# ADharaUTEXAS123007/PhysicsBasedFWI2

Hardware: AMD Instinct MI355X
Metric: grid-cells*timesteps/sec (forward+adjoint gradient pass) (higher is better)
Workload: dtype f32; 1 GPU; elastic_marmousi2_100x300_32shots_3000steps; shots_per_gpu=32, nt=3000, parallelism=shots x1, kernel_family=forward: single launch, 8 slabs/shot; adjoint: single launch, 8 slabs/shot, snapshots=f32, cells=interior

## Files before the change

### include/mifwi.h

```cpp
#ifndef MIFWI_H
#define MIFWI_H

#include <stddef.h>
#include <stdint.h>

#ifdef __cplusplus
extern "C" {
#endif

#define MIFWI_VERSION_MAJOR 0
#define MIFWI_VERSION_MINOR 7

enum {
    MIFWI_OK = 0,
    MIFWI_EINVAL = -1,
    MIFWI_ENODEVICE = -2,
    MIFWI_EHIP = -3,
    MIFWI_ECFL = -4,
    MIFWI_ENOMEM = -5
};

const char *mifwi_last_error(void);
int mifwi_version(void);
int64_t mifwi_fallback_count(void);
// ... 68 lines not shown
enum { MIFWI_SNAPSHOT_F32 = 0, MIFWI_SNAPSHOT_BF16 = 1 };

typedef struct {
    int32_t gp, pitch, ngroups, shots_per_group;
    int64_t coef_elems;
    int64_t state_elems;
    int64_t work_forward_elems;
    int64_t work_backward_elems;
    int64_t snap_step_elems;
    int32_t snapshot_format;
    int32_t kernel_flags;
} mifwi_elastic_layout;

enum { MIFWI_EL_KERNEL_FWD_SINGLE_LAUNCH = 1, MIFWI_EL_KERNEL_ADJ_SINGLE_LAUNCH = 2, MIFWI_EL_KERNEL_FWD_FUSED_STEP = 4,
       MIFWI_EL_KERNEL_ADJ_FUSED_STEP = 8,
       MIFWI_EL_KERNEL_FWD_LANE_HALO = 16, MIFWI_EL_KERNEL_ADJ_LANE_HALO = 32 };

typedef struct mifwi_elastic_plan mifwi_elastic_plan;

int mifwi_elastic_plan_create(mifwi_elastic_plan **plan, int device,
                              const mifwi_elastic_desc *desc);
int mifwi_elastic_plan_destroy(mifwi_elastic_plan *plan);
int mifwi_elastic_plan_layout(const mifwi_elastic_plan *plan, mifwi_elastic_layout *out);
int mifwi_elastic_plan_pass_sizes(const mifwi_elastic_plan *plan, int32_t *forward_shots, int32_t *adjoint_groups);

int mifwi_elastic_plan_bind_pressure(mifwi_elastic_plan *plan, float *rec_p, const float *g_p);

int mifwi_elastic_forward(mifwi_elastic_plan *plan, const float *mat, const float *pz,
                          const float *px, const float *f, const int32_t *src_cell,
                          const float *src_w, const int32_t *rec_cell, const float *rec_w,
                          float *rec_vx, float *rec_vz, float *snap, float *work, int32_t n_begin,
                          int32_t n_end, int32_t flags, void *stream);

int mifwi_elastic_backward(mifwi_elastic_plan *plan, const float *mat, const float *pz,
                           const float *px, const int32_t *src_cell, const float *src_w,
                           const int32_t *rec_cell, const float *rec_w, const float *g_vx,
                           const float *g_vz, const float *snap, int32_t snap_first,
                           float *grad_mat, float *grad_f, float *work, int32_t n_hi, int32_t n_lo,
// ... 40 lines not shown
```

### physicsbasedfwi2_amd/_lib.py

```python
import ctypes
import os

_HERE = os.path.dirname(os.path.abspath(__file__))
LIB_PATH = os.environ.get("MIFWI_LIB") or os.path.join(_HERE, "libmifwi.so")

MIFWI_OK = 0
ZERO_STATE = 1
FINALIZE = 2
_ERR_NAMES = {-1: "EINVAL", -2: "ENODEVICE", -3: "EHIP", -4: "ECFL", -5: "ENOMEM"}


class MifwiError(RuntimeError):
    pass


class AcousticDesc(ctypes.Structure):
    _fields_ = [("n0", ctypes.c_int32), ("n1", ctypes.c_int32), ("nt", ctypes.c_int32),
                ("nshot", ctypes.c_int32), ("nsrc", ctypes.c_int32), ("nrec", ctypes.c_int32),
                ("ntap", ctypes.c_int32), ("c0", ctypes.c_float), ("c1", ctypes.c_float),
                ("shots_per_group", ctypes.c_int32), ("edge_rows", ctypes.c_int32),
                ("cpml_width", ctypes.c_int32)]


class AcousticLayout(ctypes.Structure):
# ... 10 lines not shown
                ("free_surface", ctypes.c_int32), ("shots_per_group", ctypes.c_int32),
                ("source_type", ctypes.c_int32), ("record_pressure", ctypes.c_int32),
                ("snapshot_format", ctypes.c_int32), ("fd_order", ctypes.c_int32)]


class ElasticLayout(ctypes.Structure):
    _fields_ = [("gp", ctypes.c_int32), ("pitch", ctypes.c_int32), ("ngroups", ctypes.c_int32),
                ("shots_per_group", ctypes.c_int32), ("coef_elems", ctypes.c_int64),
                ("state_elems", ctypes.c_int64), ("work_forward_elems", ctypes.c_int64),
                ("work_backward_elems", ctypes.c_int64), ("snap_step_elems", ctypes.c_int64),
                ("snapshot_format", ctypes.c_int32), ("kernel_flags", ctypes.c_int32)]


EL_KERNEL_FWD_SINGLE_LAUNCH, EL_KERNEL_ADJ_SINGLE_LAUNCH, EL_KERNEL_FWD_FUSED_STEP, EL_KERNEL_ADJ_FUSED_STEP = 1, 2, 4, 8
EL_KERNEL_FWD_LANE_HALO, EL_KERNEL_ADJ_LANE_HALO = 16, 32
SNAPSHOT_F32, SNAPSHOT_BF16 = 0, 1
_P = ctypes.c_void_p

SIGNATURES = {
    "mifwi_last_error": (ctypes.c_char_p, []),
    "mifwi_version": (ctypes.c_int, []),
    "mifwi_fallback_count": (ctypes.c_int64, []),
    "mifwi_agent_handoff_count": (ctypes.c_int64, []),
    "mifwi_slow_handoff_count": (ctypes.c_int64, []),
    "mifwi_device_count": (ctypes.c_int, []),
    "mifwi_device_info": (ctypes.c_int, [ctypes.c_int, _P, _P, _P]),
    "mifwi_acoustic_plan_create": (ctypes.c_int, [ctypes.POINTER(_P), ctypes.c_int,
                                                  ctypes.POINTER(AcousticDesc)]),
    "mifwi_acoustic_plan_destroy": (ctypes.c_int, [_P]),
    "mifwi_acoustic_plan_layout": (ctypes.c_int, [_P, ctypes.POINTER(AcousticLayout)]),
    "mifwi_acoustic_forward": (ctypes.c_int, [_P] * 12 + [ctypes.c_int32] * 3 + [_P]),
    "mifwi_acoustic_backward": (ctypes.c_int, [_P] * 10 + [ctypes.c_int32] + [_P] * 3 +
                                [ctypes.c_int32] * 3 + [_P]),
    "mifwi_elastic_plan_create": (ctypes.c_int, [ctypes.POINTER(_P), ctypes.c_int,
                                                 ctypes.POINTER(ElasticDesc)]),
    "mifwi_elastic_plan_destroy": (ctypes.c_int, [_P]),
    "mifwi_elastic_plan_layout": (ctypes.c_int, [_P, ctypes.POINTER(ElasticLayout)]),
    "mifwi_elastic_plan_bind_pressure": (ctypes.c_int, [_P, _P, _P]),
    "mifwi_elastic_plan_pass_sizes": (ctypes.c_int, [_P, _P, _P]),
    "mifwi_acoustic_plan_pass_sizes": (ctypes.c_int, [_P, _P, _P]),
    "mifwi_elastic_forward": (ctypes.c_int, [_P] * 13 + [ctypes.c_int32] * 3 + [_P]),
    "mifwi_elastic_backward": (ctypes.c_int, [_P] * 11 + [ctypes.c_int32] + [_P] * 3 +
                               [ctypes.c_int32] * 3 + [_P]),
    "mifwi_acoustic_born": (ctypes.c_int, [_P] * 8 + [ctypes.c_int32] + [_P] * 2 + [ctypes.c_int32] * 3 + [_P]),
    "mifwi_acoustic_plan_cluster_slabs": (ctypes.c_int, [_P, ctypes.c_int32]),
    "mifwi_elastic_plan_cluster_slabs": (ctypes.c_int, [_P, ctypes.c_int32]),
    "mifwi_misfit_work_elems": (ctypes.c_int64, [ctypes.c_int32, ctypes.c_int64, ctypes.c_int64]),
    "mifwi_misfit": (ctypes.c_int, [ctypes.c_int, ctypes.c_int32] + [_P] * 3 + [ctypes.c_int64] * 2 +
                     [_P] * 4),
    "mifwi_gradient_condition_work_elems": (ctypes.c_int64, [ctypes.c_int32]),
    "mifwi_gradient_condition": (ctypes.c_int, [ctypes.c_int] + [_P] * 3 + [ctypes.c_int32] * 3 + [_P, ctypes.c_float] +
                                 [ctypes.c_int32] * 2 + [_P] * 3),
    "mifwi_elastic_materials": (ctypes.c_int, [ctypes.c_int] + [_P] * 4 + [ctypes.c_int32] * 2 + [ctypes.c_float, ctypes.c_int32, _P]),
    "mifwi_elastic_materials_vjp": (ctypes.c_int, [ctypes.c_int] + [_P] * 7 + [ctypes.c_int32] * 2 +
# ... 50 lines not shown
```

### physicsbasedfwi2_amd/csrc/mifwi_elastic.hip

```cpp
#include "mifwi_common.h"

#include <vector>

#include <algorithm>
#include <cmath>
#include <cstdlib>

namespace {

constexpr int kThreads = 256;
#ifndef MIFWI_EL_MINWAVES
#define MIFWI_EL_MINWAVES 1
#endif
struct FdK { float c1, c2; };
inline FdK fd_weights(int order)
{
    return order == 2 ? FdK{1.0f, 0.0f} : FdK{(float)(9.0 / 8.0), (float)(-1.0 / 24.0)};
}

enum { F_VX = 0, F_VZ = 1, F_SXX = 2, F_SZZ = 3, F_SXZ = 4 };
enum { M_L = 0, M_M = 1, M_MU = 2, M_BX = 3, M_BZ = 4 };
enum { PA = 0, PB = 1, PK = 2, PAH = 3, PBH = 4, PKH = 5 };

struct ElParams {
// ... 1013 lines not shown
    int W, wl, xr0, wx, xcd;
    float *rec_p;
    const float *g_p;
    int snap_bf16;
    long long snap_shot;
    long long splane;
    int sblk;
    int pass_shots;
    int pass_groups;
    int fused;
    int fused_pass_shots;
    long long field_stride, shot_stride, fields_elems, psix_elems, psiz_elems, coef_elems;
    long long psi_elems;
    int cluster, NW, PL, fwd_PL, adj_PL, cl_shots, cl_lds, cl_ng;
    int cl_xh, adj_xh;
    int cl_adj, adj_NW, adj_shots, adj_lds, adj_ng, adj_zrows;
    long long xbuf_elems, list_elems, xcc_elems;
    long long tile_elems;
};

namespace {

ElParams el_base(const mifwi_elastic_plan *pl, const float *mat, const float *pz, const float *px)
{
    ElParams p;
    memset(&p, 0, sizeof(p));
    p.nz = pl->d.nz; p.nx = pl->d.nx; p.ng = pl->ng; p.gp = pl->gp; p.pitch = pl->pitch;
    p.field_stride = (unsigned)pl->field_stride; p.shot_stride = pl->shot_stride;
    p.nshot = pl->d.nshot; p.gs = 1;
    p.W = pl->W; p.wl = pl->wl; p.xr0 = pl->xr0; p.wx = pl->wx;
// ... 30 lines not shown
    int extra = 0;
    if (p.smp_out0 != nullptr && p.nsmp > 0)
        extra = mifwi::ceil_div(mifwi::ceil_div(p.gs * p.nsmp, kThreads), tiles_x);
    dim3 grid(tiles_x, p.tiles_z + extra, mifwi::ceil_div(nshot, p.gs)), block(kThreads);
    switch (pl->lx) {
        case 64: hipLaunchKernelGGL((el_step_s<64, 1, SAVE>), grid, block, 0, st, p); break;
        case 32: hipLaunchKernelGGL((el_step_s<32, 1, SAVE>), grid, block, 0, st, p); break;
        default: hipLaunchKernelGGL((el_step_s<16, 1, SAVE>), grid, block, 0, st, p); break;
    }
}

void el_cluster_setup(mifwi_elastic_plan *pl)
{
    pl->cluster = 0; pl->NW = 0; pl->PL = 4 * (pl->ng + 2); pl->cl_shots = 0;
    pl->cl_xh = 0; pl->adj_xh = 0;
    pl->adj_PL = pl->PL; pl->fwd_PL = pl->PL;
    const int skew = env_int("MIFWI_EL_PL_SKEW", 1);
    int Pskew = pl->ng + 2;
    while ((Pskew - pl->ng) % 16) ++Pskew;
    const int PL_plain = pl->PL;
    if (skew & 1) pl->PL = 4 * Pskew;
    if (skew & 2) pl->adj_PL = 4 * Pskew;
    pl->cl_lds = 0; pl->xbuf_elems = 0; pl->xcc_elems = 0;
    pl->cl_adj = 0; pl->adj_NW = 0; pl->adj_shots = 0; pl->adj_lds = 0; pl->adj_ng = 0; pl->adj_zrows = 0; pl->list_elems = 0;
    {
        const long long ntiles = (long long)mifwi::ceil_div(pl->ng, AGO) * mifwi::ceil_div(pl->d.nz, ATZ);
        pl->tile_elems = std::max<long long>(1024, mifwi::round_up64(pl->d.nshot * (2 * ntiles + 1 + (long long)pl->d.nrec * pl->d.ntap), 64));
    }
    if (pl->d.ntap != 1 || pl->d.source_type != 0 || pl->d.record_pressure) return;
    const bool want_fwd = env_int("MIFWI_EL_CLUSTER", 1) != 0;
// ... 11 lines not shown
            PLq = PL_plain;
            lds = (5LL * (rows + 4) * PLq + 6LL * pl->gp + 8LL * rows + 8) * sizeof(float);
        }
        if (lds > 150 * 1024) continue;
        if ((long long)rows * pl->ng > 2 * kEcThreads || kEcRowFields * pl->gp > kEcGr * kEcThreads) continue;
        const int per_launch = 8 * (ncu / (8 * nw));
        if (per_launch < 8) break;
        const double cost = mifwi::ceil_div(pl->d.nshot, per_launch) * (4.8 + (double)rows * pl->ng / kEcThreads);
        if (cost < best - 1e-9) {
            best = cost;
            pl->cluster = 1; pl->NW = nw; pl->cl_shots = per_launch; pl->cl_lds = (int)lds;
            pl->cl_ng = mifwi::ceil_div(rows * pl->ng, kEcThreads);
            pl->fwd_PL = PLq;
        }
    }
    auto xhalo_ok = [&](int nw, int ngq) {
        if (env_int("MIFWI_EL_XHALO", 1) == 0) return 0;
        for (int w = 0; w < nw; ++w) {
            int r0, R;
            ec_slab_rows(pl->d.nz, nw, w, r0, R);
            if (!ec_xhalo_deal_ok(R, pl->ng, ngq * kEcThreads)) return 0;
        }
        return 1;
    };
    pl->cl_xh = pl->cluster ? xhalo_ok(pl->NW, pl->cl_ng) : 0;
    if (pl->cluster) {
        for (const void *fn : {(const void *)el_cluster_fwd<false, 1, false>, (const void *)el_cluster_fwd<true, 1, false>,
                               (const void *)el_cluster_fwd<false, 2, false>, (const void *)el_cluster_fwd<true, 2, false>,
                               (const void *)el_cluster_fwd<false, 1, true>, (const void *)el_cluster_fwd<true, 1, true>,
                               (const void *)el_cluster_fwd<false, 2, true>, (const void *)el_cluster_fwd<true, 2, true>,
                               (const void *)el_cluster_fwd<false, 1, false, true>, (const void *)el_cluster_fwd<true, 1, false, true>,
                               (const void *)el_cluster_fwd<false, 2, false, true>, (const void *)el_cluster_fwd<true, 2, false, true>})
            if (hipFuncSetAttribute(fn, hipFuncAttributeMaxDynamicSharedMemorySize, mifwi::kClusterLdsLimit) != hipSuccess) {
                (void)hipGetLastError();
                pl->cluster = 0;
            }
    }
    const int forced_adj = env_int("MIFWI_EL_ADJ_NW", forced);
    if (env_int("MIFWI_EL_CLUSTER_ADJ", 1) != 0 && pl->d.shots_per_group <= 0) {
        double best_adj = 1e30;
// ... 19 lines not shown
            if (lds > kEaLdsLimit && PLq != PL_plain) {
                PLq = PL_plain;
                lds = adj_lds(PLq);
            }
            if (lds > kEaLdsLimit) continue;
            if ((long long)rows * pl->ng > 2 * kEcThreads || kEcRowFields * pl->gp > kEcGr * kEcThreads) continue;
            const int per_launch = 8 * (ncu / (8 * nw));
            if (per_launch < 8) break;
            const double cost = mifwi::ceil_div(pl->d.nshot, per_launch) * (4.8 + (double)rows * pl->ng / kEcThreads);
            if (cost < best_adj - 1e-9) {
                best_adj = cost;
                pl->cl_adj = 1; pl->adj_NW = nw; pl->adj_shots = per_launch; pl->adj_lds = (int)lds; pl->adj_PL = PLq;
                pl->adj_ng = mifwi::ceil_div(rows * pl->ng, kEcThreads); pl->adj_zrows = zmax;
            }
        }
        pl->adj_xh = pl->cl_adj ? xhalo_ok(pl->adj_NW, pl->adj_ng) : 0;
        if (pl->cl_adj)
            for (const void *fn : {(const void *)el_cluster_adj<1, false>, (const void *)el_cluster_adj<2, false>,
                                   (const void *)el_cluster_adj<1, true>, (const void *)el_cluster_adj<2, true>,
                                   (const void *)el_cluster_adj<1, false, true>, (const void *)el_cluster_adj<2, false, true>})
                if (hipFuncSetAttribute(fn, hipFuncAttributeMaxDynamicSharedMemorySize, kEaLdsLimit) != hipSuccess) {
                    (void)hipGetLastError();
                    pl->cl_adj = 0;
                }
    }
    const int nwmax = std::max(pl->cluster ? pl->NW : 0, pl->cl_adj ? pl->adj_NW : 0);
    pl->xcc_elems = nwmax > 0 ? mifwi::round_up64((long long)pl->d.nshot * nwmax, 64) : 0;
    if (nwmax > 0)
        pl->xbuf_elems = mifwi::round_up64(2LL * pl->d.nshot * nwmax * 4 * kEcRowFields * pl->gp, 64) + pl->xcc_elems + 64;
    if (pl->cl_adj)
        pl->list_elems = mifwi::round_up64((long long)pl->d.nshot * pl->adj_NW * (1 + pl->d.nrec), 64);
// ... 181 lines not shown
    }
    if (pl->cl_adj) {
        pl->gs = 1;
        pl->ngroups = d->nshot;
    }
    *plan = pl;
    return MIFWI_OK;
}

int mifwi_elastic_plan_cluster_slabs(const mifwi_elastic_plan *plan, int32_t adjoint)
{
    if (!plan) return 0;
    return adjoint ? (plan->cl_adj ? plan->adj_NW : 0) : (plan->cluster ? plan->NW : 0);
}

int mifwi_elastic_plan_pass_sizes(const mifwi_elastic_plan *plan, int32_t *forward_shots, int32_t *adjoint_groups)
{
    if (!plan) return mifwi::fail(MIFWI_EINVAL, "null plan");
    if (forward_shots) *forward_shots = plan->pass_shots;
    if (adjoint_groups) *adjoint_groups = plan->pass_groups;
    return MIFWI_OK;
}

int mifwi_elastic_plan_bind_pressure(mifwi_elastic_plan *plan, float *rec_p, const float *g_p)
{
    if (!plan) return mifwi::fail(MIFWI_EINVAL, "null plan");
    if ((rec_p || g_p) && !plan->d.record_pressure)
        return mifwi::fail(MIFWI_EINVAL, "the plan was created with record_pressure = 0");
    plan->rec_p = rec_p;
    plan->g_p = g_p;
// ... 5 lines not shown
    delete plan;
    return MIFWI_OK;
}

int mifwi_elastic_plan_layout(const mifwi_elastic_plan *pl, mifwi_elastic_layout *out)
{
    if (!pl || !out) return mifwi::fail(MIFWI_EINVAL, "null plan/layout");
    out->gp = pl->gp; out->pitch = pl->pitch; out->ngroups = pl->ngroups;
    out->shots_per_group = pl->gs;
    out->coef_elems = pl->coef_elems;
    out->snap_step_elems = pl->snap_shot * pl->d.nshot;
    out->snapshot_format = pl->snap_bf16 ? MIFWI_SNAPSHOT_BF16 : MIFWI_SNAPSHOT_F32;
    out->kernel_flags = (pl->cluster ? MIFWI_EL_KERNEL_FWD_SINGLE_LAUNCH : 0) | (pl->cl_adj ? MIFWI_EL_KERNEL_ADJ_SINGLE_LAUNCH : 0) |
                        (pl->fused ? MIFWI_EL_KERNEL_FWD_FUSED_STEP : 0) |
                        (pl->cluster && pl->cl_xh ? MIFWI_EL_KERNEL_FWD_LANE_HALO : 0) |
                        (pl->cl_adj && pl->adj_xh ? MIFWI_EL_KERNEL_ADJ_LANE_HALO : 0);
    const long long psi = pl->psi_elems;
    const long long bbox = mifwi::round_up64(4LL * pl->d.nshot, 64);
    out->state_elems = pl->fields_elems + psi;
    out->work_forward_elems = out->state_elems + bbox + (pl->cluster ? pl->xbuf_elems + out->state_elems : 0) +
                              (pl->fused ? out->state_elems : 0);
    const long long adj_state = pl->fields_elems + 2 * psi + 5LL * pl->ngroups * pl->splane;
    out->work_backward_elems = adj_state + bbox + (pl->cl_adj ? pl->xbuf_elems + pl->list_elems + adj_state : 0) +
                               pl->tile_elems;
    return MIFWI_OK;
}

int mifwi_elastic_forward(mifwi_elastic_plan *pl, const float *mat, const float *pz,
                          const float *px, const float *f, const int32_t *src_cell,
                          const float *src_w, const int32_t *rec_cell, const float *rec_w,
                          float *rec_vx, float *rec_vz, float *snap, float *work, int32_t n_begin,
// ... 28 lines not shown
        EcParams c;
        memset(&c, 0, sizeof(c));
        c.nz = d.nz; c.nx = d.nx; c.ng = pl->ng; c.gp = pl->gp; c.pitch = pl->pitch;
        c.field_stride = (unsigned)pl->field_stride; c.shot_stride = pl->shot_stride;
        c.nshot = d.nshot; c.NW = pl->NW; c.PL = pl->fwd_PL;
        c.n_first = n_begin; c.n_last = n_end;
        c.W = pl->W; c.wl = pl->wl; c.xr0 = pl->xr0; c.wx = pl->wx; c.fsurf = d.free_surface;
        c.psix_shot = 4LL * d.nz * pl->wx; c.psiz_shot = 4LL * 2 * pl->W * pl->gp;
        c.mat = mat; c.pz = pz; c.px = px;
        c.fields = fields; c.psix = psi_state; c.psiz = psi_state + pl->psix_elems;
        c.S = snap; c.s_first = n_begin; c.s_step = snap_step;
        c.nsrc = d.nsrc; c.nrec = d.nrec; c.src_cell = src_cell; c.src_w = src_w; c.f = f;
        c.rec_cell = rec_cell; c.rec_w = rec_w;
        c.rec_vx = want_rec ? rec_vx : nullptr; c.rec_vz = want_rec ? rec_vz : nullptr;
        c.dbg = env_int("MIFWI_EL_CL_DBG", 0);
        c.nap = env_int("MIFWI_POLL_NAP", mifwi::ceil_div(d.nz, c.NW) >= 8 ? 48 : 1);
        c.K = fd_weights(d.fd_order);
        float *backup = xbuf + pl->xbuf_elems;
        rc = el_cluster_backup(work, pl->fields_elems + psi, backup, flags, st);
        if (rc) return rc;
        rc = snap ? el_cluster_run<true, false>(pl, c, xbuf, st) : el_cluster_run<false, false>(pl, c, xbuf, st);
        if (rc == mifwi::kClusterMisplaced) {
            mifwi::note_agent_tier("elastic forward");
            rc = el_cluster_restore(work, pl->fields_elems + psi, backup, flags, st);
            if (rc) return rc;
            rc = snap ? el_cluster_run<true, true>(pl, c, xbuf, st) : el_cluster_run<false, true>(pl, c, xbuf, st);
        }
        if (rc != mifwi::kClusterTimedOut && rc != mifwi::kClusterMisplaced) return rc;
        mifwi::note_fallback("elastic");
        rc = el_cluster_restore(work, pl->fields_elems + psi, backup, flags, st);
// ... 154 lines not shown
        c.nshot = d.nshot; c.NW = pl->adj_NW; c.PL = pl->adj_PL;
        c.n_first = n_hi; c.n_last = n_lo; c.nt = d.nt;
        c.W = pl->W; c.wl = pl->wl; c.xr0 = pl->xr0; c.wx = pl->wx; c.fsurf = d.free_surface;
        c.zrows_max = pl->adj_zrows;
        c.psix_shot = 4LL * d.nz * pl->wx; c.psiz_shot = 4LL * 2 * pl->W * pl->gp; c.psix_elems = pl->psix_elems;
        c.mat = mat; c.pz = pz; c.px = px;
        c.fields = fields; c.psiA = psiA; c.psiB = psiB;
        c.S = snap; c.s_first = snap_first; c.s_step = snap_step;
        c.acc = acc;
        c.nsrc = d.nsrc; c.nrec = d.nrec; c.src_cell = src_cell; c.src_w = src_w;
        c.grad_f = want_f ? grad_f : nullptr;
        c.rec_cell = rec_cell; c.rec_w = rec_w; c.g_vx = g_vx; c.g_vz = g_vz;
        c.slab_cnt = lists; c.slab_list = lists + (long long)d.nshot * pl->adj_NW;
        c.rcv_direct = env_int("MIFWI_EL_ADJ_DIRECT", 1);
        c.dbg = env_int("MIFWI_EL_CL_DBG", 0);
        c.nap = env_int("MIFWI_POLL_NAP", mifwi::ceil_div(d.nz, c.NW) >= 8 ? 48 : 1);
        c.K = fd_weights(d.fd_order);
        c.xbuf = reinterpret_cast<unsigned long long *>(xbuf);
        c.err = reinterpret_cast<int *>(xbuf + pl->xbuf_elems - 64);
        c.xcc_tab = reinterpret_cast<int *>(xbuf + pl->xbuf_elems - 64 - pl->xcc_elems);
        const long long adj_state = pl->fields_elems + 2 * psi + nacc;
        float *backup = reinterpret_cast<float *>(lists) + pl->list_elems;
        rc = el_cluster_backup(work, adj_state, backup, flags, st);
        if (rc) return rc;
        auto attempt = [&](bool agent) -> int {
            MIFWI_HIP_TRY(hipMemsetAsync(xbuf, 0, sizeof(float) * pl->xbuf_elems, st));
#ifdef MIFWI_ABLATIONS
            const char *trace_path = getenv("MIFWI_EL_CL_TRACE");
            const size_t trace_n = 64 * 8 * 16;
            c.trace = nullptr;
// ... 107 lines not shown
```

### physicsbasedfwi2_amd/csrc/mifwi_elastic_cluster.h

```cpp
#pragma once

constexpr int kEcThreads = 512;
constexpr unsigned kEcMaxSpin = 400000;

struct EcParams {
    int nz, nx, ng, gp, pitch;
    unsigned field_stride;
    long long shot_stride;
    int nshot, NW, PL, shot0, shot1;
    int n_first, n_last;
    int W, wl, xr0, wx, fsurf;
    long long psix_shot, psiz_shot;
    const float *mat, *pz, *px;
    float *fields, *psix, *psiz;
    float *S;
    int s_first;
    long long s_step;
    int nsrc, nrec;
    const int *src_cell;
    const float *src_w, *f;
    const int *rec_cell;
    const float *rec_w;
    float *rec_vx, *rec_vz;
    unsigned long long *xbuf;
    int *err;
    int *xcc_tab;
    int dbg, nap;
    FdK K;
#ifdef MIFWI_ABLATIONS
    long long *trace;
#endif
};

#ifdef MIFWI_ABLATIONS
#define EC_STAMP(k)                                                                                        \
    do {                                                                                                   \
        if (p.trace && tr_on && it >= 64 && it < 128 && (t & 63) == 0)                                     \
            p.trace[((it - 64) * 8 + (t >> 6)) * 16 + (k)] = (long long)__builtin_readcyclecounter();      \
    } while (0)
#define EC_LAGGARD()                                                                                       \
    do {                                                                                                   \
        if ((kDbg(p) & 4096) && w == 1 && s == p.shot0 && (it & 63) == 1)                                  \
// ... 189 lines not shown
};

#ifndef EC_LATE_INTERIOR
#define EC_LATE_INTERIOR 1
#endif
#ifndef EA_PUBLISH_FIRST
#define EA_PUBLISH_FIRST 1
#endif
#ifndef EA_MATS_AHEAD_A
#define EA_MATS_AHEAD_A 0
#endif
#ifndef EA_MATS_AHEAD_C
#define EA_MATS_AHEAD_C 1
#endif
struct EcSlot { int lrw, g, cls; };
__host__ __device__ __forceinline__ EcSlot ec_slot(int v, int R, int ng, int slots)
{
    EcSlot s;
    s.lrw = 0; s.g = 0; s.cls = 0;
#if EC_LATE_INTERIOR
    const int nint = (R > 4 ? R - 4 : 0) * ng, nb = R * ng - nint;
    int b0 = (nint + 63) & ~63;
    if (b0 + nb > slots) b0 = nint;
    if (v < nint) {
        const int ir = v / ng;
        s.lrw = 2 + ir; s.g = v - ir * ng; s.cls = v < kEcThreads ? 1 : 3;
    } else if (v >= b0 && v < b0 + nb) {
        const int bi = v - b0, br = bi / ng;
        s.g = bi - br * ng;
        s.lrw = (R > 4 && br >= 2) ? R - 4 + br : br;
        s.cls = 2;
    }
#else
    if (v < R * ng) {
        s.lrw = v / ng; s.g = v - s.lrw * ng;
        s.cls = (s.lrw >= 2 && s.lrw < R - 2) ? 1 : 2;
    }
#endif
    return s;
}

constexpr int kNbL = 1, kNbR = 2, kNbFirst = 4, kNbLast = 8;
__host__ __device__ __forceinline__ int ec_nb(int v, int R, int ng, int slots)
{
    const EcSlot s = ec_slot(v, R, ng, slots);
    if (s.cls == 0) return 0;
    const int lane = v & 63;
    const bool lv = lane != 0 && ec_slot(v - 1, R, ng, slots).cls == s.cls;
    const bool rv = lane != 63 && ec_slot(v + 1, R, ng, slots).cls == s.cls;
    return (lv ? kNbL : 0) | (rv ? kNbR : 0) | (s.g == 0 ? kNbFirst : 0) | (s.g == ng - 1 ? kNbLast : 0);
}
inline bool ec_xhalo_deal_ok(int R, int ng, int slots)
{
    for (int v = 0; v < slots; ++v) {
        const EcSlot s = ec_slot(v, R, ng, slots);
        if (s.cls == 0) continue;
        const int nb = ec_nb(v, R, ng, slots), lane = v & 63;
        if (!(nb & (kNbL | kNbR))) return false;
        const int lc = lane != 0 ? ec_slot(v - 1, R, ng, slots).cls : 0;
        if (lc >= 2 && s.cls >= 2 && lc != s.cls) return false;
    }
    return true;
}
__device__ __forceinline__ float ec_lane_below(float old, float x)
{
    return __int_as_float(__builtin_amdgcn_update_dpp(__float_as_int(old), __float_as_int(x), 0x138, 0xf, 0xf, false));
}
__device__ __forceinline__ float ec_lane_above(float old, float x)
{
    return __int_as_float(__builtin_amdgcn_update_dpp(__float_as_int(old), __float_as_int(x), 0x130, 0xf, 0xf, false));
}
template <bool XH>
__device__ __forceinline__ void ec_xhalo(const float *q, const float4 &c, const int nb, const float *dummy, float2 &L, float2 &R)
{
    if (!XH) {
// ... 216 lines not shown
    int r0, R;
    ec_slab_rows(p.nz, p.NW, w, r0, R);
    const int PL = p.PL, LR = R + 4;
    const int fsz = LR * PL;
    EcCtx c;
    for (int k = 0; k < 5; ++k) c.Lf[k] = lds + ec_plane(k) * fsz;
    float *lpx = lds + 5 * fsz, *lpz = lpx + 6 * p.gp;
    c.lpx = lpx; c.lpz = lpz; c.PL = PL; c.fsurf = p.fsurf; c.K = p.K;
    const unsigned ncell = (unsigned)p.nz * p.gp;
    const float4 zero4 = make_float4(0.f, 0.f, 0.f, 0.f);
    const long long xplane = (long long)p.nz * p.wx, zplane = 2LL * p.W * p.gp;
    auto strip_x = [&](int g) { const int c0 = 4 * g; return p.W <= 0 ? -1 : c0 < p.wl ? c0 : c0 >= p.xr0 ? p.wl + (c0 - p.xr0) : -1; };
    auto strip_z = [&](int j) { return p.W <= 0 ? -1 : j < p.W ? j : j >= p.nz - p.W ? j - (p.nz - 2 * p.W) : -1; };

    EcGroup G[NG];
    bool slow = p.nrec > kEcThreads;
    int tsq = -1;
    unsigned tsrc4 = 0;
    unsigned tm0 = 0, tm1 = 0, tm2 = 0, tm3 = 0;
    float tw = 0.f, tnext = 0.f;
    int src_mask = 0;
#pragma unroll
    for (int q = 0; q < NG; ++q) {
        EcGroup &g = G[q];
        const EcSlot sl = ec_slot(t + q * kEcThreads, R, p.ng, NG * kEcThreads);
        const bool own = sl.cls != 0;
        const int lrw = sl.lrw;
        g.g = sl.g;
        g.j = r0 + lrw;
        g.cls = sl.cls;
        g.nb = XH ? ec_nb(t + q * kEcThreads, R, p.ng, NG * kEcThreads) : 0;
        g.lo = (lrw + 2) * PL + 4 + 4 * g.g;
        const unsigned gcc = (unsigned)g.j * p.gp + 4 * g.g;
        g.gcb = 4u * gcc;
        g.mL = g.mM = g.mMu = g.mBx = g.mBz = zero4;
        g.s1 = g.s2 = g.s3 = g.s4 = g.s5 = g.s6 = g.s7 = g.s8 = zero4;
        g.xtab = -1; g.ztab = -1;
        int xs_off = -1, zs = -1;
        if (own) {
            g.mL = ld4(p.mat + M_L * ncell + gcc); g.mM = ld4(p.mat + M_M * ncell + gcc);
            g.mMu = ld4(p.mat + M_MU * ncell + gcc);
            g.mBx = ld4(p.mat + M_BX * ncell + gcc); g.mBz = ld4(p.mat + M_BZ * ncell + gcc);
            xs_off = strip_x(g.g); zs = strip_z(g.j);
        }
        if (xs_off >= 0) {
            g.xtab = 24 * g.g;
            const float *q = p.psix + (long long)s * p.psix_shot + (long long)g.j * p.wx + xs_off;
            g.s1 = ld4(q); g.s3 = ld4(q + xplane); g.s5 = ld4(q + 2 * xplane); g.s8 = ld4(q + 3 * xplane);
        }
        if (zs >= 0) {
            g.ztab = 8 * lrw;
            const float *q = p.psiz + (long long)s * p.psiz_shot + (long long)zs * p.gp + 4 * g.g;
            g.s2 = ld4(q); g.s4 = ld4(q + zplane); g.s6 = ld4(q + 2 * zplane); g.s7 = ld4(q + 3 * zplane);
        }
        for (int e = 0; e < p.nsrc; ++e) {
            const int cell = p.src_cell[(long long)s * p.nsrc + e];
            if (cell < 0) continue;
            const int i0 = cell / p.nx, i1 = cell - i0 * p.nx;
            if (own && i0 == g.j && (i1 >> 2) == g.g) {
                if (tsq >= 0) slow = true;
                tw = p.src_w[(long long)s * p.nsrc + e];
                tsq = q; tsrc4 = 4u * e;
                tm0 = (i1 & 3) == 0 ? ~0u : 0u; tm1 = (i1 & 3) == 1 ? ~0u : 0u;
// ... 235 lines not shown
    int s_first;
    long long s_step;
    float *acc;
    int nsrc, nrec;
    const int *src_cell;
    const float *src_w;
    float *grad_f;
    const int *rec_cell;
    const float *rec_w, *g_vx, *g_vz;
    const int *slab_cnt, *slab_list;
    int rcv_direct;
    unsigned long long *xbuf;
    int *err;
    int *xcc_tab;
    int dbg, nap;
    FdK K;
#ifdef MIFWI_ABLATIONS
    long long *trace;
#endif
};

__global__ void ec_build_slab_lists(const int *rec_cell, int nrec, int nz, int nx, int NW, int *slab_cnt,
                                    int *slab_list)
{
    const int s = blockIdx.x;
    __shared__ int cnt[64];
    if ((int)threadIdx.x < NW) cnt[threadIdx.x] = 0;
    __syncthreads();
    const int base = nz / NW, rem = nz - base * NW;
    for (int e = threadIdx.x; e < nrec; e += blockDim.x) {
// ... 52 lines not shown
    const long long xplane = (long long)p.nz * p.wx, zplane = 2LL * p.W * p.gp;
    const int ztop_end = p.W > 0 ? min(r0 + R, p.W) : r0;
    const int ntop = max(0, ztop_end - r0);
    const int zbot_beg = p.W > 0 ? max(r0, p.nz - p.W) : r0 + R;
    const int zrows = ntop + max(0, r0 + R - zbot_beg);
    const int xsz = R * p.wx, zsz = zrows * p.gp;
    const int PL_ = PL, fsz_ = fsz, xsz_ = xsz, zsz_ = zsz;
    const unsigned ncell_ = ncell;

    const int par_in = (p.nt - 1 - p.n_first) & 1;
    const float *psi_in = par_in ? p.psiB : p.psiA;
    const int par_out = (p.nt - 1 - (p.n_last - 1)) & 1;
    float *psi_out = par_out ? p.psiB : p.psiA;

    EaGroup G[NG];
    bool slow = false;
#pragma unroll
    for (int q = 0; q < NG; ++q) {
        EaGroup &g = G[q];
        const EcSlot sl = ec_slot(t + q * kEcThreads, R, p.ng, NG * kEcThreads);
        const bool own = sl.cls != 0;
        const int lrw = sl.lrw;
        g.g = sl.g;
        g.j = r0 + lrw;
        g.lo = (lrw + 2) * PL + 4 + 4 * g.g;
        g.cls = sl.cls;
        g.nb = XH ? ec_nb(t + q * kEcThreads, R, p.ng, NG * kEcThreads) : 0;
        g.bxx = g.bzz = g.bxz = g.vx = g.vz = zero4;
        g.a0 = g.a1 = g.a2 = g.a3 = g.a4 = zero4;
        g.S1 = g.S2 = g.S3 = g.S4 = g.S5 = zero4;
        g.xsl = -1; g.zsl = -1; g.src = -1; g.src_wt = 0.f;
        if (own) {
            const unsigned gcc = (unsigned)g.j * p.gp + 4 * g.g;
            const long long o = (long long)(g.j + 2) * p.pitch + 4 + 4 * g.g;
            const float *gf = p.fields + (long long)s * p.shot_stride;
            g.vx = ld4(gf + F_VX * p.field_stride + o); g.vz = ld4(gf + F_VZ * p.field_stride + o);
            g.bxx = ld4(gf + F_SXX * p.field_stride + o); g.bzz = ld4(gf + F_SZZ * p.field_stride + o);
            g.bxz = ld4(gf + F_SXZ * p.field_stride + o);
            const float *ga = p.acc + (long long)s * 5 * ncell + gcc;
            g.a0 = ld4(ga); g.a1 = ld4(ga + ncell); g.a2 = ld4(ga + 2 * (long long)ncell);
            g.a3 = ld4(ga + 3 * (long long)ncell); g.a4 = ld4(ga + 4 * (long long)ncell);
            if (p.W > 0) {
                const int c0 = 4 * g.g;
                int xs_off = -1, zs = -1;
                if (c0 < p.wl) xs_off = c0; else if (c0 >= p.xr0) xs_off = p.wl + (c0 - p.xr0);
                if (g.j < p.W) zs = g.j; else if (g.j >= p.nz - p.W) zs = g.j - (p.nz - 2 * p.W);
                if (xs_off >= 0) {
                    g.xsl = lrw * p.wx + xs_off;
                    const float *qx = psi_in + (long long)s * p.psix_shot + (long long)g.j * p.wx + xs_off;
#pragma unroll
                    for (int k = 0; k < 4; ++k) st4(lxs + k * xsz + g.xsl, ld4(qx + k * xplane));
                }
                if (zs >= 0) {
                    const int zl = (g.j < p.W) ? g.j - r0 : ntop + (g.j - zbot_beg);
                    g.zsl = zl * p.gp + 4 * g.g;
                    const float *qz = psi_in + p.psix_elems + (long long)s * p.psiz_shot + (long long)zs * p.gp + 4 * g.g;
#pragma unroll
                    for (int k = 0; k < 4; ++k) st4(lzs + k * zsz + g.zsl, ld4(qz + k * zplane));
                }
            }
        }
        if (p.grad_f != nullptr)
            for (int e = 0; e < p.nsrc; ++e) {
                const int cell = p.src_cell[(long long)s * p.nsrc + e];
                if (cell < 0) continue;
                const int i0 = cell / p.nx, i1 = cell - i0 * p.nx;
// ... 510 lines not shown
```

Before: 68760 Mcells*steps/s.

## Deal PML strip groups into separate wavefront segments in cluster kernels

```diff
diff --git a/include/mifwi.h b/include/mifwi.h
--- a/include/mifwi.h
+++ b/include/mifwi.h
@@ -106,7 +106,8 @@
 
 enum { MIFWI_EL_KERNEL_FWD_SINGLE_LAUNCH = 1, MIFWI_EL_KERNEL_ADJ_SINGLE_LAUNCH = 2, MIFWI_EL_KERNEL_FWD_FUSED_STEP = 4,
        MIFWI_EL_KERNEL_ADJ_FUSED_STEP = 8,
-       MIFWI_EL_KERNEL_FWD_LANE_HALO = 16, MIFWI_EL_KERNEL_ADJ_LANE_HALO = 32 };
+       MIFWI_EL_KERNEL_FWD_LANE_HALO = 16, MIFWI_EL_KERNEL_ADJ_LANE_HALO = 32,
+       MIFWI_EL_KERNEL_FWD_STRIP_DEAL = 64, MIFWI_EL_KERNEL_ADJ_STRIP_DEAL = 128 };
 
 typedef struct mifwi_elastic_plan mifwi_elastic_plan;
 
@@ -114,6 +115,8 @@
                               const mifwi_elastic_desc *desc);
 int mifwi_elastic_plan_destroy(mifwi_elastic_plan *plan);
 int mifwi_elastic_plan_layout(const mifwi_elastic_plan *plan, mifwi_elastic_layout *out);
+int mifwi_elastic_deal_table(int32_t rows, int32_t groups, int32_t strip_left, int32_t strip_right, int32_t group_slots,
+                             int32_t mode, int32_t *table, int32_t *lane_halo_ok);
 int mifwi_elastic_plan_pass_sizes(const mifwi_elastic_plan *plan, int32_t *forward_shots, int32_t *adjoint_groups);
 
 int mifwi_elastic_plan_bind_pressure(mifwi_elastic_plan *plan, float *rec_p, const float *g_p);
diff --git a/physicsbasedfwi2_amd/_lib.py b/physicsbasedfwi2_amd/_lib.py
--- a/physicsbasedfwi2_amd/_lib.py
+++ b/physicsbasedfwi2_amd/_lib.py
@@ -48,6 +48,7 @@
 
 EL_KERNEL_FWD_SINGLE_LAUNCH, EL_KERNEL_ADJ_SINGLE_LAUNCH, EL_KERNEL_FWD_FUSED_STEP, EL_KERNEL_ADJ_FUSED_STEP = 1, 2, 4, 8
 EL_KERNEL_FWD_LANE_HALO, EL_KERNEL_ADJ_LANE_HALO = 16, 32
+EL_KERNEL_FWD_STRIP_DEAL, EL_KERNEL_ADJ_STRIP_DEAL = 64, 128
 SNAPSHOT_F32, SNAPSHOT_BF16 = 0, 1
 _P = ctypes.c_void_p
 
@@ -72,6 +73,7 @@
     "mifwi_elastic_plan_layout": (ctypes.c_int, [_P, ctypes.POINTER(ElasticLayout)]),
     "mifwi_elastic_plan_bind_pressure": (ctypes.c_int, [_P, _P, _P]),
     "mifwi_elastic_plan_pass_sizes": (ctypes.c_int, [_P, _P, _P]),
+    "mifwi_elastic_deal_table": (ctypes.c_int, [ctypes.c_int32] * 6 + [_P, _P]),
     "mifwi_acoustic_plan_pass_sizes": (ctypes.c_int, [_P, _P, _P]),
     "mifwi_elastic_forward": (ctypes.c_int, [_P] * 13 + [ctypes.c_int32] * 3 + [_P]),
     "mifwi_elastic_backward": (ctypes.c_int, [_P] * 11 + [ctypes.c_int32] + [_P] * 3 +
diff --git a/physicsbasedfwi2_amd/csrc/mifwi_elastic.hip b/physicsbasedfwi2_amd/csrc/mifwi_elastic.hip
--- a/physicsbasedfwi2_amd/csrc/mifwi_elastic.hip
+++ b/physicsbasedfwi2_amd/csrc/mifwi_elastic.hip
@@ -1051,6 +1051,8 @@
     long long psi_elems;
     int cluster, NW, PL, fwd_PL, adj_PL, cl_shots, cl_lds, cl_ng;
     int cl_xh, adj_xh;
+    int cl_deal, adj_deal;
+    int cl_seg, adj_seg;
     int cl_adj, adj_NW, adj_shots, adj_lds, adj_ng, adj_zrows;
     long long xbuf_elems, list_elems, xcc_elems;
     long long tile_elems;
@@ -1111,6 +1113,7 @@
 {
     pl->cluster = 0; pl->NW = 0; pl->PL = 4 * (pl->ng + 2); pl->cl_shots = 0;
     pl->cl_xh = 0; pl->adj_xh = 0;
+    pl->cl_deal = pl->adj_deal = pl->cl_seg = pl->adj_seg = 0;
     pl->adj_PL = pl->PL; pl->fwd_PL = pl->PL;
     const int skew = env_int("MIFWI_EL_PL_SKEW", 1);
     int Pskew = pl->ng + 2;
@@ -1152,16 +1155,27 @@
             pl->fwd_PL = PLq;
         }
     }
-    auto xhalo_ok = [&](int nw, int ngq) {
+    auto slab_deal = [&](int nw, int w, int ngq, int mode) {
+        int r0, R, gl, gr;
+        ec_slab_rows(pl->d.nz, nw, w, r0, R);
+        ec_strip_groups(pl->W, pl->wl, pl->xr0, pl->ng, mode, gl, gr);
+        return ec_deal(R, pl->ng, gl, gr, ngq * kEcThreads, mode);
+    };
+    auto xhalo_ok = [&](int nw, int ngq, int mode) {
         if (env_int("MIFWI_EL_XHALO", 1) == 0) return 0;
-        for (int w = 0; w < nw; ++w) {
-            int r0, R;
-            ec_slab_rows(pl->d.nz, nw, w, r0, R);
-            if (!ec_xhalo_deal_ok(R, pl->ng, ngq * kEcThreads)) return 0;
-        }
+        for (int w = 0; w < nw; ++w)
+            if (!ec_xhalo_deal_ok(slab_deal(nw, w, ngq, mode))) return 0;
         return 1;
     };
-    pl->cl_xh = pl->cluster ? xhalo_ok(pl->NW, pl->cl_ng) : 0;
+    auto pick_deal = [&](int nw, int ngq, int dflt, int &mode, int &xh, int &seg) {
+        mode = std::min(2, std::max(0, env_int("MIFWI_EL_DEAL", dflt)));
+        xh = xhalo_ok(nw, ngq, mode);
+        if (mode && !xh && xhalo_ok(nw, ngq, 0)) { mode = 0; xh = 1; }
+        seg = 0;
+        for (int w = 0; w < nw; ++w)
+            if (slab_deal(nw, w, ngq, mode).level > 0) seg = 1;
+    };
+    if (pl->cluster) pick_deal(pl->NW, pl->cl_ng, 0, pl->cl_deal, pl->cl_xh, pl->cl_seg);
     if (pl->cluster) {
         for (const void *fn : {(const void *)el_cluster_fwd<false, 1, false>, (const void *)el_cluster_fwd<true, 1, false>,
                                (const void *)el_cluster_fwd<false, 2, false>, (const void *)el_cluster_fwd<true, 2, false>,
@@ -1211,7 +1225,7 @@
                 pl->adj_ng = mifwi::ceil_div(rows * pl->ng, kEcThreads); pl->adj_zrows = zmax;
             }
         }
-        pl->adj_xh = pl->cl_adj ? xhalo_ok(pl->adj_NW, pl->adj_ng) : 0;
+        if (pl->cl_adj) pick_deal(pl->adj_NW, pl->adj_ng, 1, pl->adj_deal, pl->adj_xh, pl->adj_seg);
         if (pl->cl_adj)
             for (const void *fn : {(const void *)el_cluster_adj<1, false>, (const void *)el_cluster_adj<2, false>,
                                    (const void *)el_cluster_adj<1, true>, (const void *)el_cluster_adj<2, true>,
@@ -1423,6 +1437,22 @@
     return adjoint ? (plan->cl_adj ? plan->adj_NW : 0) : (plan->cluster ? plan->NW : 0);
 }
 
+int mifwi_elastic_deal_table(int32_t rows, int32_t groups, int32_t strip_left, int32_t strip_right, int32_t group_slots,
+                             int32_t mode, int32_t *table, int32_t *lane_halo_ok)
+{
+    if (rows < 1 || groups < 1 || strip_left < 0 || strip_right < 0 || group_slots < 1 || group_slots > 2 || !table ||
+        (long long)rows * groups > (long long)group_slots * kEcThreads)
+        return mifwi::fail(MIFWI_EINVAL, "bad deal shape %dx%d on %d group slots", rows, groups, group_slots);
+    const EcDeal d = ec_deal(rows, groups, strip_left, strip_right, group_slots * kEcThreads, mode);
+    for (int v = 0; v < d.slots; ++v) {
+        const EcSlot s = ec_slot(v, d);
+        table[4 * v] = s.cls ? s.lrw : -1; table[4 * v + 1] = s.cls ? s.g : -1;
+        table[4 * v + 2] = s.cls; table[4 * v + 3] = ec_nb(v, d);
+    }
+    if (lane_halo_ok) *lane_halo_ok = ec_xhalo_deal_ok(d) ? 1 : 0;
+    return d.level;
+}
+
 int mifwi_elastic_plan_pass_sizes(const mifwi_elastic_plan *plan, int32_t *forward_shots, int32_t *adjoint_groups)
 {
     if (!plan) return mifwi::fail(MIFWI_EINVAL, "null plan");
@@ -1458,7 +1488,9 @@
     out->kernel_flags = (pl->cluster ? MIFWI_EL_KERNEL_FWD_SINGLE_LAUNCH : 0) | (pl->cl_adj ? MIFWI_EL_KERNEL_ADJ_SINGLE_LAUNCH : 0) |
                         (pl->fused ? MIFWI_EL_KERNEL_FWD_FUSED_STEP : 0) |
                         (pl->cluster && pl->cl_xh ? MIFWI_EL_KERNEL_FWD_LANE_HALO : 0) |
-                        (pl->cl_adj && pl->adj_xh ? MIFWI_EL_KERNEL_ADJ_LANE_HALO : 0);
+                        (pl->cl_adj && pl->adj_xh ? MIFWI_EL_KERNEL_ADJ_LANE_HALO : 0) |
+                        (pl->cluster && pl->cl_seg ? MIFWI_EL_KERNEL_FWD_STRIP_DEAL : 0) |
+                        (pl->cl_adj && pl->adj_seg ? MIFWI_EL_KERNEL_ADJ_STRIP_DEAL : 0);
     const long long psi = pl->psi_elems;
     const long long bbox = mifwi::round_up64(4LL * pl->d.nshot, 64);
     out->state_elems = pl->fields_elems + psi;
@@ -1517,6 +1549,7 @@
         c.rec_cell = rec_cell; c.rec_w = rec_w;
         c.rec_vx = want_rec ? rec_vx : nullptr; c.rec_vz = want_rec ? rec_vz : nullptr;
         c.dbg = env_int("MIFWI_EL_CL_DBG", 0);
+        c.deal = pl->cl_deal;
         c.nap = env_int("MIFWI_POLL_NAP", mifwi::ceil_div(d.nz, c.NW) >= 8 ? 48 : 1);
         c.K = fd_weights(d.fd_order);
         float *backup = xbuf + pl->xbuf_elems;
@@ -1701,6 +1734,7 @@
         c.slab_cnt = lists; c.slab_list = lists + (long long)d.nshot * pl->adj_NW;
         c.rcv_direct = env_int("MIFWI_EL_ADJ_DIRECT", 1);
         c.dbg = env_int("MIFWI_EL_CL_DBG", 0);
+        c.deal = pl->adj_deal;
         c.nap = env_int("MIFWI_POLL_NAP", mifwi::ceil_div(d.nz, c.NW) >= 8 ? 48 : 1);
         c.K = fd_weights(d.fd_order);
         c.xbuf = reinterpret_cast<unsigned long long *>(xbuf);
diff --git a/physicsbasedfwi2_amd/csrc/mifwi_elastic_cluster.h b/physicsbasedfwi2_amd/csrc/mifwi_elastic_cluster.h
--- a/physicsbasedfwi2_amd/csrc/mifwi_elastic_cluster.h
+++ b/physicsbasedfwi2_amd/csrc/mifwi_elastic_cluster.h
@@ -26,6 +26,7 @@
     int *err;
     int *xcc_tab;
     int dbg, nap;
+    int deal;
     FdK K;
 #ifdef MIFWI_ABLATIONS
     long long *trace;
@@ -245,11 +246,61 @@
 #define EA_MATS_AHEAD_C 1
 #endif
 struct EcSlot { int lrw, g, cls; };
-__host__ __device__ __forceinline__ EcSlot ec_slot(int v, int R, int ng, int slots)
-{
+struct EcDeal {
+    int R, ng, gl, gr, slots;
+    int level;
+    int is0, b0, bs0;
+};
+__host__ __device__ __forceinline__ EcDeal ec_deal(int R, int ng, int gl, int gr, int slots, int mode)
+{
+    EcDeal d;
+    d.R = R; d.ng = ng; d.gl = gl; d.gr = gr; d.slots = slots;
+    d.level = 0; d.is0 = d.b0 = d.bs0 = 0;
+    const int nn = ng - gl - gr, ns = gl + gr, ri = R - 4;
+    if (mode <= 0 || ns <= 0 || nn < 2 || ri < 1) return d;
+    d.is0 = (ri * (nn + 1) - 1 + 63) & ~63;
+    d.b0 = (d.is0 + ri * (ns + 1) + 63) & ~63;
+    const int bn = 4 * (nn + 1) - 1, bs = 4 * (ns + 1);
+    const int nint = ri * ng, nbnd = 4 * ng;
+    const int plain = ((nint + 63) & ~63) + nbnd <= slots ? ((nint + 63) >> 6) + ((nbnd + 63) >> 6) : (nint + nbnd + 63) >> 6;
+    const int ws3 = (((d.b0 + bn + 63) & ~63) + bs + 63) >> 6, ws2 = (d.b0 + bn + 1 + bs + 63) >> 6, ws1 = (d.b0 + nbnd + 63) >> 6;
+    if (mode >= 2 && ws3 <= plain && ws3 * 64 <= slots) { d.level = 3; d.bs0 = (d.b0 + bn + 63) & ~63; }
+    else if (mode >= 2 && ws2 <= plain && ws2 * 64 <= slots) { d.level = 2; d.bs0 = d.b0 + bn + 1; }
+    else if (ws1 <= plain && ws1 * 64 <= slots) d.level = 1;
+    return d;
+}
+__host__ __device__ __forceinline__ EcSlot ec_slot(int v, const EcDeal &d)
+{
+    const int R = d.R, ng = d.ng, slots = d.slots;
     EcSlot s;
     s.lrw = 0; s.g = 0; s.cls = 0;
+    if (v < 0 || v >= slots) return s;
 #if EC_LATE_INTERIOR
+    if (d.level > 0) {
+        const int nn = ng - d.gl - d.gr, ns = d.gl + d.gr, ri = R - 4;
+        int row = -1, g = 0;
+        if (v < d.is0) {
+            const int r = v / (nn + 1), k = v - r * (nn + 1);
+            if (r < ri && k < nn) { row = r; g = d.gl + k; }
+        } else if (v < d.b0) {
+            const int u = v - d.is0, r = u / (ns + 1), k = u - r * (ns + 1);
+            if (r < ri && k != d.gl) { row = r; g = k < d.gl ? k : ng - d.gr + (k - d.gl - 1); }
+        } else if (d.level == 1) {
+            const int u = v - d.b0, r = u / ng;
+            if (r < 4) { row = ri + r; g = u - r * ng; }
+        } else if (v < d.bs0) {
+            const int u = v - d.b0, r = u / (nn + 1), k = u - r * (nn + 1);
+            if (r < 4 && k < nn) { row = ri + r; g = d.gl + k; }
+        } else {
+            const int u = v - d.bs0, r = u / (ns + 1), k = u - r * (ns + 1);
+            if (r < 4 && k != d.gl) { row = ri + r; g = k < d.gl ? k : ng - d.gr + (k - d.gl - 1); }
+        }
+        if (row < 0) return s;
+        s.g = g;
+        if (row < ri) { s.lrw = 2 + row; s.cls = v < kEcThreads ? 1 : 3; }
+        else { const int br = row - ri; s.lrw = br >= 2 ? R - 4 + br : br; s.cls = 2; }
+        return s;
+    }
     const int nint = (R > 4 ? R - 4 : 0) * ng, nb = R * ng - nint;
     int b0 = (nint + 63) & ~63;
     if (b0 + nb > slots) b0 = nint;
@@ -270,26 +321,38 @@
 #endif
     return s;
 }
+__host__ __device__ __forceinline__ void ec_strip_groups(int W, int wl, int xr0, int ng, int mode, int &gl, int &gr)
+{
+    gl = gr = 0;
+    if (W > 0 && mode != 0) { gl = (wl + 3) / 4; gr = ng - xr0 / 4; }
+}
 
 constexpr int kNbL = 1, kNbR = 2, kNbFirst = 4, kNbLast = 8;
-__host__ __device__ __forceinline__ int ec_nb(int v, int R, int ng, int slots)
-{
-    const EcSlot s = ec_slot(v, R, ng, slots);
+__host__ __device__ __forceinline__ bool ec_adjacent(const EcSlot &a, const EcSlot &b, int ng)
+{
+    return (a.lrw == b.lrw && a.g + 1 == b.g) || (a.g == ng - 1 && b.g == 0);
+}
+__host__ __device__ __forceinline__ int ec_nb(int v, const EcDeal &d)
+{
+    const EcSlot s = ec_slot(v, d);
     if (s.cls == 0) return 0;
     const int lane = v & 63;
-    const bool lv = lane != 0 && ec_slot(v - 1, R, ng, slots).cls == s.cls;
-    const bool rv = lane != 63 && ec_slot(v + 1, R, ng, slots).cls == s.cls;
-    return (lv ? kNbL : 0) | (rv ? kNbR : 0) | (s.g == 0 ? kNbFirst : 0) | (s.g == ng - 1 ? kNbLast : 0);
-}
-inline bool ec_xhalo_deal_ok(int R, int ng, int slots)
-{
-    for (int v = 0; v < slots; ++v) {
-        const EcSlot s = ec_slot(v, R, ng, slots);
+    const EcSlot lo = ec_slot(v - 1, d), hi = ec_slot(v + 1, d);
+    const bool lv = lane != 0 && lo.cls == s.cls && ec_adjacent(lo, s, d.ng);
+    const bool rv = lane != 63 && hi.cls == s.cls && ec_adjacent(s, hi, d.ng);
+    return (lv ? kNbL : 0) | (rv ? kNbR : 0) | (s.g == 0 ? kNbFirst : 0) | (s.g == d.ng - 1 ? kNbLast : 0);
+}
+inline bool ec_xhalo_deal_ok(const EcDeal &d)
+{
+    for (int v = 0; v < d.slots; ++v) {
+        const EcSlot s = ec_slot(v, d);
         if (s.cls == 0) continue;
-        const int nb = ec_nb(v, R, ng, slots), lane = v & 63;
+        const int nb = ec_nb(v, d), lane = v & 63;
         if (!(nb & (kNbL | kNbR))) return false;
-        const int lc = lane != 0 ? ec_slot(v - 1, R, ng, slots).cls : 0;
-        if (lc >= 2 && s.cls >= 2 && lc != s.cls) return false;
+        if (lane == 0) continue;
+        const EcSlot lo = ec_slot(v - 1, d);
+        if (lo.cls >= 2 && s.cls >= 2 && lo.cls != s.cls) return false;
+        if (lo.cls == s.cls && !ec_adjacent(lo, s, d.ng)) return false;
     }
     return true;
 }
@@ -536,6 +599,9 @@
     auto strip_z = [&](int j) { return p.W <= 0 ? -1 : j < p.W ? j : j >= p.nz - p.W ? j - (p.nz - 2 * p.W) : -1; };
 
     EcGroup G[NG];
+    int dgl, dgr;
+    ec_strip_groups(p.W, p.wl, p.xr0, p.ng, p.deal, dgl, dgr);
+    const EcDeal deal = ec_deal(R, p.ng, dgl, dgr, NG * kEcThreads, p.deal);
     bool slow = p.nrec > kEcThreads;
     int tsq = -1;
     unsigned tsrc4 = 0;
@@ -545,13 +611,13 @@
 #pragma unroll
     for (int q = 0; q < NG; ++q) {
         EcGroup &g = G[q];
-        const EcSlot sl = ec_slot(t + q * kEcThreads, R, p.ng, NG * kEcThreads);
+        const EcSlot sl = ec_slot(t + q * kEcThreads, deal);
         const bool own = sl.cls != 0;
         const int lrw = sl.lrw;
         g.g = sl.g;
         g.j = r0 + lrw;
         g.cls = sl.cls;
-        g.nb = XH ? ec_nb(t + q * kEcThreads, R, p.ng, NG * kEcThreads) : 0;
+        g.nb = XH ? ec_nb(t + q * kEcThreads, deal) : 0;
         g.lo = (lrw + 2) * PL + 4 + 4 * g.g;
         const unsigned gcc = (unsigned)g.j * p.gp + 4 * g.g;
         g.gcb = 4u * gcc;
@@ -569,6 +635,7 @@
             g.xtab = 24 * g.g;
             const float *q = p.psix + (long long)s * p.psix_shot + (long long)g.j * p.wx + xs_off;
             g.s1 = ld4(q); g.s3 = ld4(q + xplane); g.s5 = ld4(q + 2 * xplane); g.s8 = ld4(q + 3 * xplane);
+            if (kDbg(p) & 8192) g.xtab = -1;
         }
         if (zs >= 0) {
             g.ztab = 8 * lrw;
@@ -834,6 +901,7 @@
     int *err;
     int *xcc_tab;
     int dbg, nap;
+    int deal;
     FdK K;
 #ifdef MIFWI_ABLATIONS
     long long *trace;
@@ -916,18 +984,21 @@
     float *psi_out = par_out ? p.psiB : p.psiA;
 
     EaGroup G[NG];
+    int dgl, dgr;
+    ec_strip_groups(p.W, p.wl, p.xr0, p.ng, p.deal, dgl, dgr);
+    const EcDeal deal = ec_deal(R, p.ng, dgl, dgr, NG * kEcThreads, p.deal);
     bool slow = false;
 #pragma unroll
     for (int q = 0; q < NG; ++q) {
         EaGroup &g = G[q];
-        const EcSlot sl = ec_slot(t + q * kEcThreads, R, p.ng, NG * kEcThreads);
+        const EcSlot sl = ec_slot(t + q * kEcThreads, deal);
         const bool own = sl.cls != 0;
         const int lrw = sl.lrw;
         g.g = sl.g;
         g.j = r0 + lrw;
         g.lo = (lrw + 2) * PL + 4 + 4 * g.g;
         g.cls = sl.cls;
-        g.nb = XH ? ec_nb(t + q * kEcThreads, R, p.ng, NG * kEcThreads) : 0;
+        g.nb = XH ? ec_nb(t + q * kEcThreads, deal) : 0;
         g.bxx = g.bzz = g.bxz = g.vx = g.vz = zero4;
         g.a0 = g.a1 = g.a2 = g.a3 = g.a4 = zero4;
         g.S1 = g.S2 = g.S3 = g.S4 = g.S5 = zero4;
@@ -952,6 +1023,7 @@
                     const float *qx = psi_in + (long long)s * p.psix_shot + (long long)g.j * p.wx + xs_off;
 #pragma unroll
                     for (int k = 0; k < 4; ++k) st4(lxs + k * xsz + g.xsl, ld4(qx + k * xplane));
+                    if (kDbg(p) & 8192) g.xsl = -1;
                 }
                 if (zs >= 0) {
                     const int zl = (g.j < p.W) ? g.j - r0 : ntop + (g.j - zbot_beg);
```

Result: faster. 70380 Mcells*steps/s, median of 6 (+2.4%).
